# ly27253/LED-Net

Measured on AMD Instinct MI355X. Metric: images/sec at 1024x1024, LED-Net fwd+bwd, higher is better.
Workload: dtype bf16; 1 GPU; LED-Net 1024x1024 train_step (fwd+OHEM-CE+bwd+SGD) batch 16/GPU; global_batch=16, parallelism=dp1, ranks=1, batchnorm=per-rank statistics, submission=hipGraph replay, deterministic=False

## Files before the change

include/ledn.h:

```cpp
#ifndef LEDN_H
#define LEDN_H

#ifdef __cplusplus
extern "C" {
#endif

#define LEDN_ABI_VERSION 5

enum { LEDN_OK = 0, LEDN_EINVAL = 1, LEDN_ELAUNCH = 2, LEDN_ESKIP = 3  };
enum { LEDN_F32 = 0, LEDN_BF16 = 1, LEDN_U8 = 2 };
enum { LEDN_ACT_NONE = 0, LEDN_ACT_RELU = 1, LEDN_ACT_RELU6 = 2, LEDN_ACT_PRELU = 3, LEDN_ACT_SIGMOID = 4 };
enum { LEDN_RES_NONE = 0, LEDN_RES_ADD = 1, LEDN_RES_GATE = 2 };

int ledn_abi_version(void);

int ledn_set_workspace(void* ptr, long long nfloats);
int ledn_bind_workspace(void* stream, void* ptr, long long nfloats);

enum {
    LEDN_OPT_CONV_WORKGROUPS = 0,
    LEDN_OPT_WGRAD_WORKGROUPS = 1,
    LEDN_OPT_STREAM_FAST = 2,
    LEDN_OPT_BN_FUSED = 4,
    LEDN_OPT_DETERMINISTIC = 3
};
int ledn_set_option(int option, long long value);

typedef struct {
    const void* x;
    const void* xadd;
    const float* w;
    const void* w_bf16;
    void* y;
    const void* res;
    const float* in_scale;
    const float* in_shift;
    const float* out_scale;
    const float* out_shift;
    const float* slope;
    float* stat_sum;
    float* stat_sqsum;
    long long ws_co, ws_ci, ws_tap;
    int N, H, W, Cin, Ho, Wo, Cout;
    int KH, KW, stride, pad, dil, groups;
    int in_act, act_out, res_mode;
    int dtype_x, dtype_y;
    int transposed;
    const float* in_slope;
} ledn_conv_desc;
int ledn_conv2d(const ledn_conv_desc* d, void* stream);
int ledn_conv2d_deferred_stats(const ledn_conv_desc* d, float** part, int* rows, void* stream);
int ledn_stats_defer_begin(void);
int ledn_stats_defer_end(float** part, int* rows);
int ledn_conv2d_uses_mfma(const ledn_conv_desc* d);

int ledn_pack_conv_weights(const float* w, void* out_bf16, int Cout, int Cin, int KH, int KW, int mode,
// ... 242 lines not shown
int ledn_bn_act_bwd_reduce(const ledn_bnbwd_desc* d, void* stream);
int ledn_bn_act_bwd_apply(const ledn_bnbwd_desc* d, void* stream);
int ledn_bn_act_bwd_fused(const ledn_bnbwd_desc* d, void* stream);
int ledn_bn_act_bwd_fused_check(int C, void* stream);

typedef struct {
    ledn_bnbwd_desc bn;
    const void* head_dz;
    const float* w;
    float* dw;
    float* db;
    int N, H, W, Co;
    int dtype_dz;
} ledn_headbwd_desc;
int ledn_head_bwd_supported(const ledn_headbwd_desc* d);
int ledn_head_bwd_reduce(const ledn_headbwd_desc* d, void* stream);
int ledn_head_bwd_apply(const ledn_headbwd_desc* d, void* stream);

typedef struct {
    const void* x;
    const void* dz;
    const float* w;
    const void* add;
    void* dx;
    float* dw;
    int N, H, W, C, Ho, Wo;
    int KH, KW, stride, pad;
    int dil[4], group_size;
    int ext1;
    int dtype;
} ledn_dwbwd_desc;
int ledn_dwconv2d_bwd_data(const ledn_dwbwd_desc* d, void* stream);
int ledn_dwconv2d_bwd_weight(const ledn_dwbwd_desc* d, void* stream);

typedef struct {
    const void* x;
    const void* dy;
    const float* w;
    void* gsum;
    void* dx;
    float* dw;
    int N, H, W, n, Ho, Wo, stride;
    int dil[4];
    int dtype;
} ledn_pyrbwd_desc;
int ledn_sesp_pyramid_bwd_data(const ledn_pyrbwd_desc* d, void* stream);
int ledn_sesp_pyramid_bwd_weight(const ledn_pyrbwd_desc* d, void* stream);
int ledn_sesp_pyramid_bwd_kernel_id(const ledn_pyrbwd_desc* d);

int ledn_bilinear_bwd(const void* dy, void* dx, int N, int H, int W, int C, int Ho, int Wo,
                      int dtype_dy, int dtype_dx, void* stream);
int ledn_avgpool3x3s2_bwd(const void* dy, const void* add, void* dx, int N, int H, int W, int C,
                          int Ho, int Wo, int dtype, void* stream);

int ledn_window_attn_bwd(const void* qkv, const float* biasT, const void* dout, float* dqkv,
                         float* dbiasT, int N, int H, int W, int C, int heads, int ws, int dtype,
                         void* stream);
int ledn_getb_pool_bwd(const void* dout, void* da, int N, int H, int W, int C, int ws, int dtype,
                       void* stream);

typedef struct {
    const void* x;
    const void* r;
    const void* xl;
    const float* ctx[4];
    int ctx_size[4];
// ... 244 lines not shown
```

led-net_amd/_lib.py:

```python
import contextlib
import ctypes as C
import os

_HERE = os.path.dirname(os.path.abspath(__file__))
from ._env import knob as _knob
HIP_LIB_PATH = _knob('LEDN_HIP_LIB', None) or os.path.join(_HERE, 'csrc', 'libledn_hip.so')

OK, EINVAL, ELAUNCH = 0, 1, 2
F32, BF16, U8 = 0, 1, 2
ACT_NONE, ACT_RELU, ACT_RELU6, ACT_PRELU, ACT_SIGMOID = 0, 1, 2, 3, 4
RES_NONE, RES_ADD, RES_GATE = 0, 1, 2
OPT_CONV_WORKGROUPS, OPT_WGRAD_WORKGROUPS, OPT_STREAM_FAST, OPT_DETERMINISTIC, OPT_BN_FUSED = 0, 1, 2, 3, 4
ESKIP = 3

vp, fp, i32, i64 = C.c_void_p, C.c_void_p, C.c_int, C.c_longlong


class ConvDesc(C.Structure):
    _fields_ = [('x', vp), ('xadd', vp), ('w', fp), ('w_bf16', vp), ('y', vp), ('res', vp),
                ('in_scale', fp), ('in_shift', fp), ('out_scale', fp), ('out_shift', fp),
                ('slope', fp), ('stat_sum', fp), ('stat_sqsum', fp),
                ('ws_co', i64), ('ws_ci', i64), ('ws_tap', i64),
                ('N', i32), ('H', i32), ('W', i32), ('Cin', i32), ('Ho', i32), ('Wo', i32), ('Cout', i32),
                ('KH', i32), ('KW', i32), ('stride', i32), ('pad', i32), ('dil', i32), ('groups', i32),
                ('in_act', i32), ('act_out', i32), ('res_mode', i32),
                ('dtype_x', i32), ('dtype_y', i32), ('transposed', i32), ('in_slope', fp)]


class WgradDesc(C.Structure):
    _fields_ = [('x', vp), ('xadd', vp), ('dz', vp), ('dw', fp), ('db', fp),
                ('in_scale', fp), ('in_shift', fp),
                ('ws_co', i64), ('ws_ci', i64), ('ws_tap', i64),
                ('N', i32), ('H', i32), ('W', i32), ('Cin', i32), ('Ho', i32), ('Wo', i32), ('Cout', i32),
                ('KH', i32), ('KW', i32), ('stride', i32), ('pad', i32), ('dil', i32), ('groups', i32),
                ('in_act', i32), ('dtype_x', i32), ('dtype_dz', i32), ('in_slope', fp)]


class WgradFinishEntry(C.Structure):
    _fields_ = [('part', fp), ('dw', fp), ('ws_co', i64), ('ws_ci', i64), ('ws_tap', i64),
                ('nbx', i32), ('pairs', i32), ('KK', i32), ('ci_tiles', i32), ('Cin', i32), ('Cout', i32),
                ('groups', i32), ('chunk0', i32)]


class DwDesc(C.Structure):
    _fields_ = [('x', vp), ('w', fp), ('y', vp), ('out_scale', fp), ('out_shift', fp), ('slope', fp),
# ... 113 lines not shown
    _fields_ = [('w', fp), ('out', vp), ('Cout', i32), ('Cin', i32), ('KK', i32), ('mode', i32), ('groups', i32)]


class SgdEntry(C.Structure):
    _fields_ = [('p', fp), ('g', fp), ('m', fp), ('n', i64)]


class OptimEntry(C.Structure):
    _fields_ = [('p', fp), ('g', fp), ('m', fp), ('v', fp), ('n', i64), ('lr_mult', C.c_float), ('wd_mult', C.c_float)]


class EmaEntry(C.Structure):
    _fields_ = [('avg', fp), ('src', fp), ('n', i64)]


class OptimDesc(C.Structure):
    _fields_ = [('kind', i32), ('has_v', i32), ('lr_a', C.c_float), ('lr_b', C.c_float), ('sched_dev', fp),
                ('momentum', C.c_float), ('eps', C.c_float), ('beta1', C.c_double), ('beta2', C.c_double),
                ('bc1', C.c_float), ('sqrt_bc2', C.c_float), ('weight_decay', C.c_float), ('grad_scale', C.c_float),
                ('clip', i32), ('norm_type', i32), ('partials', fp), ('n_partials', i32), ('max_norm', C.c_float),
                ('clip_value', C.c_float), ('norm_out', fp)]


_PROTOS = {
    'ledn_bn_act_bwd_reduce': ([C.POINTER(BnBwdDesc), vp], i32),
    'ledn_bn_act_bwd_apply': ([C.POINTER(BnBwdDesc), vp], i32),
    'ledn_head_bwd_supported': ([C.POINTER(HeadBwdDesc)], i32),
    'ledn_head_bwd_reduce': ([C.POINTER(HeadBwdDesc), vp], i32),
    'ledn_head_bwd_apply': ([C.POINTER(HeadBwdDesc), vp], i32),
    'ledn_bn_act_bwd_fused': ([C.POINTER(BnBwdDesc), vp], i32),
    'ledn_bn_act_bwd_fused_check': ([i32, vp], i32),
    'ledn_dwconv2d_bwd_data': ([C.POINTER(DwBwdDesc), vp], i32),
    'ledn_dwconv2d_bwd_weight': ([C.POINTER(DwBwdDesc), vp], i32),
    'ledn_sesp_pyramid_bwd_data': ([C.POINTER(PyrBwdDesc), vp], i32),
    'ledn_sesp_pyramid_bwd_weight': ([C.POINTER(PyrBwdDesc), vp], i32),
    'ledn_sesp_pyramid_bwd_kernel_id': ([C.POINTER(PyrBwdDesc)], i32),
    'ledn_bilinear_bwd': ([vp, vp, i32, i32, i32, i32, i32, i32, i32, i32, vp], i32),
    'ledn_avgpool3x3s2_bwd': ([vp, vp, vp, i32, i32, i32, i32, i32, i32, i32, vp], i32),
    'ledn_window_attn_bwd': ([vp, fp, vp, fp, fp, i32, i32, i32, i32, i32, i32, i32, vp], i32),
    'ledn_getb_pool_bwd': ([vp, vp, i32, i32, i32, i32, i32, i32, vp], i32),
    'ledn_mfaf_gate_bwd': ([C.POINTER(MfafBwdDesc), vp], i32),
    'ledn_mfaf_bwd_combine': ([vp, vp, vp, C.POINTER(fp), C.POINTER(i32), i32, i32, i32, i32, i32, i32, vp], i32),
    'ledn_ohem_work_floats': ([i64], i64),
    'ledn_ohem_ce_fwd': ([fp, vp, i64, i32, C.c_float, i64, C.c_float, i32, fp, fp, vp], i32),
    'ledn_ohem_ce_bwd': ([fp, vp, i64, i32, i32, fp, fp, fp, C.c_float, fp, vp], i32),
    'ledn_ohem_ce_up_fwd': ([fp, i32, i32, i32, i32, i32, vp, C.c_float, i64, C.c_float, i32, fp, fp, vp], i32),
    'ledn_ohem_ce_up_bwd': ([fp, i32, i32, i32, i32, i32, vp, i32, fp, fp, fp, C.c_float, fp, vp], i32),
    'ledn_ohem2_up_fwd': ([fp, fp, i32, i32, i32, i32, i32, vp, C.c_float, i64, C.c_float, C.c_float, i64, C.c_float, i32,
                           fp, fp, vp], i32),
    'ledn_ohem2_up_bwd': ([fp, fp, i32, i32, i32, i32, i32, i32, fp, fp, fp, fp, C.c_float, C.c_float, fp, fp, vp], i32),
    'ledn_ohem2_work_floats': ([i64], i64),
    'ledn_ohem_ce_w_fwd': ([fp, vp, i64, i32, C.c_float, i64, C.c_float, i32, fp, fp, fp, vp], i32),
    'ledn_ohem_ce_w_bwd': ([fp, vp, i64, i32, i32, fp, fp, fp, C.c_float, fp, fp, vp], i32),
    'ledn_ohem_ce_up_w_fwd': ([fp, i32, i32, i32, i32, i32, vp, C.c_float, i64, C.c_float, i32, fp, fp, fp, vp], i32),
    'ledn_ohem_ce_up_w_bwd': ([fp, i32, i32, i32, i32, i32, vp, i32, fp, fp, fp, C.c_float, fp, fp, vp], i32),
    'ledn_ohem2_up_w_fwd': ([fp, fp, i32, i32, i32, i32, i32, vp, C.c_float, i64, C.c_float, C.c_float, i64, C.c_float, i32,
                             fp, fp, fp, fp, vp], i32),
    'ledn_ohem2_up_w_bwd': ([fp, fp, i32, i32, i32, i32, i32, i32, fp, fp, fp, fp, C.c_float, C.c_float, fp, fp, fp, fp,
                             vp], i32),
    'ledn_seg_loss_work_floats': ([i64], i64),
    'ledn_ce_loss_fwd': ([fp, vp, i32, i64, i32, fp, i32, i32, i32, C.c_float, fp, fp, vp], i32),
    'ledn_ce_loss_bwd': ([fp, vp, i32, i64, i32, fp, i32, C.c_float, fp, fp, fp, fp, vp], i32),
    'ledn_ce_loss_up_fwd': ([fp, i32, i32, i32, i32, i32, vp, fp, i32, i32, i32, C.c_float, fp, fp, vp], i32),
    'ledn_ce_loss_up_bwd': ([fp, i32, i32, i32, i32, i32, vp, fp, i32, C.c_float, fp, fp, fp, fp, vp], i32),
    'ledn_dice_loss_fwd': ([fp, vp, i32, i64, i32, i32, i32, i32, i32, i32, C.c_float, C.c_float, fp, fp, vp], i32),
    'ledn_dice_loss_bwd': ([fp, vp, i32, i64, i32, i32, i32, i32, i32, C.c_float, C.c_float, fp, fp, fp, fp, vp], i32),
# ... 167 lines not shown
```

led-net_amd/csrc/backward.hip:

```cpp
#include "ledn_rt.h"
#include "stencil.h"

namespace ledn {

template <int V>
struct BnParams {
    float sc[V], sh[V], sl[V], mean[V], invstd[V];
};

template <int V>
__device__ __forceinline__ BnParams<V> bn_params(const ledn_bnbwd_desc& d, int c) {
    BnParams<V> p;
#pragma unroll
    for (int i = 0; i < V; ++i) {
        p.sc[i] = d.scale ? d.scale[c + i] : 1.f;
        p.sh[i] = d.shift ? d.shift[c + i] : 0.f;
        p.sl[i] = d.slope ? d.slope[c + i] : 0.f;
        p.mean[i] = d.bn_mode ? d.mean[c + i] : 0.f;
        p.invstd[i] = d.bn_mode ? d.invstd[c + i] : 0.f;
    }
    return p;
}

template <int V>
// ... 563 lines not shown
        if (!part && nbx > 64) {
            ppb = cdiv(cdiv(npix, 64), rows) * rows;
            nbx = cdiv(npix, ppb);
        }
        const dim3 g8((unsigned)nbx, (unsigned)d.KH);
        if (d.dtype == LEDN_F32) LEDN_LAUNCH((dw_bwd_weight_row_kernel<float, 4, 8>), g8, dim3(256), 0, s, d, (int)ppb, part);
        else if (d.dtype == LEDN_BF16) LEDN_LAUNCH((dw_bwd_weight_row_kernel<bf16_t, 4, 8>), g8, dim3(256), 0, s, d, (int)ppb, part);
        else return LEDN_EINVAL;
        if (part) return finish_partials(part, (int)nbx, d.KH * 8 * d.C, 1, d.dw, nullptr, nullptr, s);
        return check_launch();
    }
    const int taps = d.KH * d.KW;
    long ppb = cdiv(npix * taps, 8192);
    if (ppb < 128) ppb = 128;
    long nbx = cdiv(npix, ppb);
    float* part = (nbx > 8 || det()) ? ws_take(nbx * taps * d.C) : nullptr;
    if (!part) {
        ppb = cdiv(npix * taps, 2048);
        if (ppb < 128) ppb = 128;
        nbx = cdiv(npix, ppb);
    }
    const dim3 grid((unsigned)nbx, (unsigned)taps);
#define LEDN_K(T)                                                                                       \
    do {                                                                                                \
        if (v4) LEDN_LAUNCH((dw_bwd_weight_kernel<T, 4>), grid, dim3(256), 0, s, d, (int)ppb, part);    \
        else LEDN_LAUNCH((dw_bwd_weight_kernel<T, 1>), grid, dim3(256), 0, s, d, (int)ppb, part);       \
    } while (0)
    if (d.dtype == LEDN_F32) LEDN_K(float);
    else if (d.dtype == LEDN_BF16) LEDN_K(bf16_t);
    else return LEDN_EINVAL;
#undef LEDN_K
    if (part) return finish_partials(part, (int)nbx, taps * d.C, 1, d.dw, nullptr, nullptr, s);
    return check_launch();
}

template <typename T, int V>
__global__ void __launch_bounds__(256) pyr_suffix_kernel(const T* dy, T* g, long npix, int n) {
    const int cv = n / V;
    const long idx = (long)blockIdx.x * blockDim.x + threadIdx.x;
    if (idx >= npix * cv) return;
    const int c = (int)(idx % cv) * V;
    const long pix = idx / cv;
    float run[V];
#pragma unroll
    for (int v = 0; v < V; ++v) run[v] = 0.f;
    for (int b = 3; b >= 0; --b) {
        float t[V];
        ldv<V>(dy + pix * 4L * n + (long)b * n + c, t);
#pragma unroll
        for (int v = 0; v < V; ++v) run[v] += t[v];
        stv<V>(g + pix * 4L * n + (long)b * n + c, run);
    }
}

template <typename T, int V>
__global__ void __launch_bounds__(256) pyr_bwd_data_kernel(ledn_pyrbwd_desc d) {
    const int cv = d.n / V;
    const long total = (long)d.N * d.H * d.W * cv;
    const long idx = (long)xcd_block(blockIdx.x, gridDim.x) * blockDim.x + threadIdx.x;
    if (idx >= total) return;
    const NhwcIdx ix_ = nhwc_split(idx, cv, d.W, d.H);
    const int c = ix_.cv * V;
    const long pix = ix_.pix;
    const int x = ix_.x, y = ix_.y, n = ix_.n;
    const T* g = reinterpret_cast<const T*>(d.gsum);
    float acc[V];
// ... 800 lines not shown
```

led-net_amd/csrc/capi.hip:

```cpp
#include "ledn_rt.h"

namespace ledn {
int conv_validate(const ledn_conv_desc& d);
int conv_direct(const ledn_conv_desc& d, hipStream_t s);
bool conv_mfma_supported(const ledn_conv_desc& d);
bool conv_f32_mfma_supported(const ledn_conv_desc& d);
int conv_f32_mfma(const ledn_conv_desc& d, hipStream_t s);
bool conv_wgrad_f32_mfma_supported(const ledn_wgrad_desc& d);
int conv_wgrad_f32_mfma(const ledn_wgrad_desc& d, hipStream_t s);
int conv_mfma(const ledn_conv_desc& d, hipStream_t s);
int conv_wgrad_mfma_partial(const ledn_wgrad_desc& d, float* part, long long part_floats, ledn_wgrad_finish_entry* entry,
                            bool query, hipStream_t s);
int conv_wgrad_finish_multi_impl(const ledn_wgrad_finish_entry* table_dev, int n, int total_chunks, hipStream_t s);
bool conv1x1_reg_supported(const ledn_conv_desc& d);
int conv1x1_reg(const ledn_conv_desc& d, hipStream_t s);
bool conv3x3_reg_supported(const ledn_conv_desc& d);
int conv3x3_reg(const ledn_conv_desc& d, hipStream_t s);
bool conv3x3_narrowin_mfma_supported(const ledn_conv_desc& d);
int conv3x3_narrowin_mfma(const ledn_conv_desc& d, hipStream_t s);
bool wgrad_mfma_supported(const ledn_wgrad_desc& d);
bool conv_wgrad_cout2_supported(const ledn_wgrad_desc& d);
bool conv_wgrad_narrow_reg_supported(const ledn_wgrad_desc& d);
bool conv1x1_wgrad_reg_applies(const ledn_wgrad_desc& d);
int conv_wgrad_narrow_reg(const ledn_wgrad_desc& d, hipStream_t s);
// ... 34 lines not shown
int channel_stats_impl(const void* x, const void* xadd, long long P, int C, int dtype, float* sum,
                       float* sqsum, hipStream_t s);
int bn_finalize_impl(const float* sum, const float* sqsum, double count, const float* gamma,
                     const float* beta, float* running_mean, float* running_var, float momentum,
                     float eps, float* scale, float* shift, float* mean, float* invstd, int C,
                     hipStream_t s);
int affine_act_impl(const ledn_affine_desc& d, hipStream_t s);
int bilinear_impl(const ledn_resize_desc& d, hipStream_t s);
int nchw_to_nhwc_impl(const void* x, int dtype_x, void* y, int dtype_y, int N, int C, int H, int W,
                      const float* scale, const float* shift, const int* map, const int* valid_hw, float pad_val,
                      hipStream_t s);
int avgpool2d_impl(const void* x, void* y, int N, int H, int W, int C, int Ho, int Wo, int k, int st, int pad,
                   int dtype, hipStream_t s);
int avgpool2d_bwd_impl(const void* dy, void* dx, int N, int H, int W, int C, int Ho, int Wo, int k, int st, int pad,
                       int dtype, hipStream_t s);
int relpos_bias_impl(const float* table, const long long* index, float* out, int R, int heads, int T, hipStream_t s);
int relpos_bias_bwd_impl(const float* dbias, const long long* index, float* dtable, int R, int heads, int T,
                         hipStream_t s);
int adaptive_avgpool_impl(const void* x, const void* xadd, float* y, int N, int H, int W, int C, int S,
                          int dtype, hipStream_t s);
int avgpool3x3s2_impl(const void* x, void* y, int N, int H, int W, int C, int Ho, int Wo, int dtype,
                      hipStream_t s);
int window_attn_impl(const void* qkv, const float* biasT, void* out, int N, int H, int W, int C,
                     int heads, int ws, int dtype, hipStream_t s);
int getb_pool_impl(const void* a, const void* local, void* out, int N, int H, int W, int C, int ws,
                   int dtype, hipStream_t s);
int mfaf_gate_impl(const ledn_mfaf_desc& d, hipStream_t s);
int seam_edge_impl(const float* seg, float* edge, float* scratch, int N, int h, int w, int kth, float thr,
                   float final_thr, hipStream_t s);
int bn_act_bwd_reduce_impl(const ledn_bnbwd_desc& d, hipStream_t s);
int bn_act_bwd_apply_impl(const ledn_bnbwd_desc& d, hipStream_t s);
int dw_bwd_data_impl(const ledn_dwbwd_desc& d, hipStream_t s);
int dw_bwd_weight_impl(const ledn_dwbwd_desc& d, hipStream_t s);
int pyr_bwd_data_impl(const ledn_pyrbwd_desc& d, hipStream_t s);
int pyr_bwd_weight_impl(const ledn_pyrbwd_desc& d, hipStream_t s);
int pyr_bwd_data_kernel_id(const ledn_pyrbwd_desc& d);
int bilinear_bwd_impl(const void* dy, void* dx, int N, int H, int W, int C, int Ho, int Wo, int dtype_dy,
                      int dtype_dx, hipStream_t s);
int avgpool3x3s2_bwd_impl(const void* dy, const void* add, void* dx, int N, int H, int W, int C, int Ho,
                          int Wo, int dtype, hipStream_t s);
int window_attn_bwd_impl(const void* qkv, const float* biasT, const void* dout, float* dqkv, float* dbiasT,
                         int N, int H, int W, int C, int heads, int ws, int dtype, hipStream_t s);
int getb_pool_bwd_impl(const void* dout, void* da, int N, int H, int W, int C, int ws, int dtype,
                       hipStream_t s);
int mfaf_gate_bwd_impl(const ledn_mfafbwd_desc& d, hipStream_t s);
int mfaf_bwd_combine_impl(void* dx, void* dr, const void* dxl, const float* const* dpool, const int* sizes,
                          int npool, int N, int H, int W, int C, int dtype, hipStream_t s);
long long ohem_work_floats(long long P);
int ohem_ce_fwd_impl(const float* logits, const long long* target, long long P, int C, float thres,
                     long long min_kept, float loss_weight, int ignore_label, const float* cw, float* work,
                     float* out, hipStream_t s);
int ohem_ce_up_fwd_impl(const float* src, int N, int Hs, int Ws, int H, int W, const long long* target, float thres,
                        long long min_kept, float loss_weight, int ignore_label, const float* cw, float* work,
                        float* out, hipStream_t s);
int ohem2_up_fwd_impl(const float* src0, const float* src1, int N, int Hs, int Ws, int H, int W,
                      const long long* target, float thres0, long long min_kept0, float lw0, float thres1,
                      long long min_kept1, float lw1, int ignore_label, const float* cw0, const float* cw1,
                      float* work, float* out, hipStream_t s);
int ohem2_up_bwd_impl(const float* src0, const float* src1, int N, int Hs, int Ws, int H, int W, int ignore_label,
                      const float* work, const float* out, const float* dloss0, const float* dloss1, float lw0,
                      float lw1, const float* cw0, const float* cw1, float* dsrc0, float* dsrc1, hipStream_t s);
long long ohem2_work_floats(long long P);
int ohem_ce_up_bwd_impl(const float* src, int N, int Hs, int Ws, int H, int W, const long long* target,
                        int ignore_label, const float* work, const float* out, const float* dloss, float loss_weight,
                        const float* cw, float* dsrc, hipStream_t s);
int ohem_ce_bwd_impl(const float* logits, const long long* target, long long P, int C, int ignore_label,
// ... 20 lines not shown
int slide_accumulate_impl(float* canvas, const float* crop, int N, int C, int H, int W, int y1, int x1, int hc, int wc,
                          int crop_planar, hipStream_t s);
int slide_finish_impl(float* canvas, const int* rowcnt, const int* colcnt, unsigned char* mask, int N, int C, int H,
                      int W, hipStream_t s);
int sgd_step_impl(const ledn_sgd_entry* table_dev, int n_tensors, long long max_n, float lr,
                  const float* lr_dev, float momentum, float weight_decay, float grad_scale, hipStream_t s);
int grad_norm_partials_impl(const float* g, long long n, int norm_type, float* partials, int n_partials, hipStream_t s);
int sgd_step_clip_impl(const ledn_sgd_entry* table_dev, int n_tensors, long long max_n, float lr, const float* lr_dev,
                       float momentum, float weight_decay, float grad_scale, const float* partials, int n_partials,
                       int norm_type, float max_norm, float clip_value, float* norm_out, hipStream_t s);
int optim_step_impl(const ledn_optim_entry* table_dev, int n_tensors, long long max_n, const ledn_optim_desc* d, hipStream_t s);
int optim_step_ema_impl(const ledn_optim_entry* table_dev, float* const* avg_table_dev, int n_tensors, long long max_n,
                        const ledn_optim_desc* d, float w, const float* w_dev, hipStream_t s);
int ema_update_impl(const ledn_ema_entry* table_dev, int n_tensors, long long max_n, float w, const float* w_dev, hipStream_t s);
}

#include <mutex>
#include <unordered_map>

namespace ledn {
static Workspace g_ws = {nullptr, 0};
static std::mutex g_ws_mutex;
static std::unordered_map<void*, Workspace> g_ws_by_stream;
static thread_local void* tls_stream = nullptr;
static thread_local Workspace tls_ws = {nullptr, 0};
static hipStream_t enter_stream(void* stream) {
    tls_stream = stream;
    std::lock_guard<std::mutex> lock(g_ws_mutex);
    auto it = g_ws_by_stream.find(stream);
    tls_ws = it != g_ws_by_stream.end() ? it->second : g_ws;
    return (hipStream_t)stream;
}
Workspace& workspace() { return tls_ws; }
static Options g_opt = {512, 512, 91, 0, 0};
Options& options() { return g_opt; }
static thread_local DeferredStats g_defer = {false, nullptr, 0};
DeferredStats& deferred_stats() { return g_defer; }
}

using namespace ledn;
#define S(stream) (ledn::enter_stream(stream))

extern "C" {

int ledn_abi_version(void) { return LEDN_ABI_VERSION; }

int ledn_set_workspace(void* ptr, long long nfloats) {
    if (nfloats < 0 || (ptr == nullptr) != (nfloats == 0)) return LEDN_EINVAL;
    std::lock_guard<std::mutex> lock(g_ws_mutex);
    g_ws = Workspace{(float*)ptr, (long)nfloats};
    if (g_ws_by_stream.find(tls_stream) == g_ws_by_stream.end()) tls_ws = g_ws;
    return LEDN_OK;
}

int ledn_bind_workspace(void* stream, void* ptr, long long nfloats) {
    if (nfloats < 0 || (ptr == nullptr) != (nfloats == 0)) return LEDN_EINVAL;
    std::lock_guard<std::mutex> lock(g_ws_mutex);
    if (ptr) g_ws_by_stream[stream] = Workspace{(float*)ptr, (long)nfloats};
    else g_ws_by_stream.erase(stream);
    return LEDN_OK;
}

int ledn_set_option(int option, long long value) {
    if (value > (1 << 20)) return LEDN_EINVAL;
    switch (option) {
        case LEDN_OPT_CONV_WORKGROUPS: options().conv_workgroups = value > 0 ? (int)value : 512; return LEDN_OK;
        case LEDN_OPT_WGRAD_WORKGROUPS: options().wgrad_workgroups = value > 0 ? (int)value : 512; return LEDN_OK;
        case LEDN_OPT_STREAM_FAST: options().stream_fast = value < 0 ? 91 : (int)value; return LEDN_OK;
        case LEDN_OPT_DETERMINISTIC: options().deterministic = value > 0 ? 1 : 0; return LEDN_OK;
        case LEDN_OPT_BN_FUSED: options().bn_fused = value > 0 ? 1 : 0; return LEDN_OK;
        default: return LEDN_EINVAL;
    }
}

int ledn_conv2d(const ledn_conv_desc* d, void* stream) {
    if (!d) return LEDN_EINVAL;
    const int rc = conv_validate(*d);
    if (rc != LEDN_OK) return rc;
    if (head_fwd_supported(*d)) return head_fwd(*d, S(stream));
    if (head_mc_conv_kind(*d)) return head_mc_conv(*d, S(stream));
    if (conv_mfma_supported(*d)) {
        if (conv1x1_reg_supported(*d)) return conv1x1_reg(*d, S(stream));
        if (conv3x3_reg_supported(*d)) return conv3x3_reg(*d, S(stream));
        return conv_mfma(*d, S(stream));
    }
    if (conv3x3_narrowin_mfma_supported(*d)) return conv3x3_narrowin_mfma(*d, S(stream));
    if (conv_f32_mfma_supported(*d)) return conv_f32_mfma(*d, S(stream));
    return conv_direct(*d, S(stream));
}

int ledn_stats_defer_begin(void) {
    DeferredStats& ds = deferred_stats();
    ds.want = true;
    ds.part = nullptr;
    ds.rows = 0;
    return LEDN_OK;
}
int ledn_stats_defer_end(float** part, int* rows) {
    if (!part || !rows) return LEDN_EINVAL;
    DeferredStats& ds = deferred_stats();
    *part = ds.part;
    *rows = ds.part ? ds.rows : 0;
    ds.want = false;
// ... 226 lines not shown
int ledn_mfaf_gate(const ledn_mfaf_desc* d, void* stream) { return d ? mfaf_gate_impl(*d, S(stream)) : LEDN_EINVAL; }
int ledn_seam_edge(const float* seg, float* edge, float* scratch, int N, int h, int w, int kth, float thr,
                   float final_thr, void* stream) {
    return seam_edge_impl(seg, edge, scratch, N, h, w, kth, thr, final_thr, S(stream));
}

int ledn_bn_act_bwd_reduce(const ledn_bnbwd_desc* d, void* stream) {
    return d ? bn_act_bwd_reduce_impl(*d, S(stream)) : LEDN_EINVAL;
}
int ledn_bn_act_bwd_apply(const ledn_bnbwd_desc* d, void* stream) {
    return d ? bn_act_bwd_apply_impl(*d, S(stream)) : LEDN_EINVAL;
}
int ledn_bn_act_bwd_fused(const ledn_bnbwd_desc* d, void* stream) {
    if (!d) return LEDN_EINVAL;
    if (!options().bn_fused) return LEDN_ESKIP;
    return bn_act_bwd_fused(*d, S(stream));
}
int ledn_bn_act_bwd_fused_check(int C, void* stream) { return bn_act_bwd_fused_check(C, S(stream)); }
int ledn_head_bwd_supported(const ledn_headbwd_desc* d) { return d ? head_bwd_supported(*d) : 0; }
int ledn_head_bwd_reduce(const ledn_headbwd_desc* d, void* stream) {
    LEDN_REQUIRE(d);
    return head_bwd_reduce(*d, S(stream));
}
int ledn_head_bwd_apply(const ledn_headbwd_desc* d, void* stream) {
    LEDN_REQUIRE(d);
    return head_bwd_apply(*d, S(stream));
}
int ledn_dwconv2d_bwd_data(const ledn_dwbwd_desc* d, void* stream) {
    return d ? dw_bwd_data_impl(*d, S(stream)) : LEDN_EINVAL;
}
int ledn_dwconv2d_bwd_weight(const ledn_dwbwd_desc* d, void* stream) {
    return d ? dw_bwd_weight_impl(*d, S(stream)) : LEDN_EINVAL;
}
int ledn_sesp_pyramid_bwd_data(const ledn_pyrbwd_desc* d, void* stream) {
    return d ? pyr_bwd_data_impl(*d, S(stream)) : LEDN_EINVAL;
}
int ledn_sesp_pyramid_bwd_weight(const ledn_pyrbwd_desc* d, void* stream) {
    return d ? pyr_bwd_weight_impl(*d, S(stream)) : LEDN_EINVAL;
}
int ledn_sesp_pyramid_bwd_kernel_id(const ledn_pyrbwd_desc* d) { return d ? pyr_bwd_data_kernel_id(*d) : -1; }
int ledn_bilinear_bwd(const void* dy, void* dx, int N, int H, int W, int C, int Ho, int Wo, int dtype_dy,
                      int dtype_dx, void* stream) {
    return bilinear_bwd_impl(dy, dx, N, H, W, C, Ho, Wo, dtype_dy, dtype_dx, S(stream));
}
int ledn_avgpool3x3s2_bwd(const void* dy, const void* add, void* dx, int N, int H, int W, int C, int Ho,
                          int Wo, int dtype, void* stream) {
    return avgpool3x3s2_bwd_impl(dy, add, dx, N, H, W, C, Ho, Wo, dtype, S(stream));
}
int ledn_window_attn_bwd(const void* qkv, const float* biasT, const void* dout, float* dqkv, float* dbiasT,
                         int N, int H, int W, int C, int heads, int ws, int dtype, void* stream) {
    return window_attn_bwd_impl(qkv, biasT, dout, dqkv, dbiasT, N, H, W, C, heads, ws, dtype, S(stream));
}
int ledn_getb_pool_bwd(const void* dout, void* da, int N, int H, int W, int C, int ws, int dtype,
                       void* stream) {
    return getb_pool_bwd_impl(dout, da, N, H, W, C, ws, dtype, S(stream));
}
int ledn_mfaf_gate_bwd(const ledn_mfafbwd_desc* d, void* stream) {
    return d ? mfaf_gate_bwd_impl(*d, S(stream)) : LEDN_EINVAL;
}
int ledn_mfaf_bwd_combine(void* dx, void* dr, const void* dxl, const float* const* dpool, const int* sizes,
                          int npool, int N, int H, int W, int C, int dtype, void* stream) {
    return mfaf_bwd_combine_impl(dx, dr, dxl, dpool, sizes, npool, N, H, W, C, dtype, S(stream));
}
long long ledn_ohem_work_floats(long long P) { return ohem_work_floats(P); }
int ledn_ohem_ce_fwd(const float* logits, const long long* target, long long P, int C, float thres,
                     long long min_kept, float loss_weight, int ignore_label, float* work, float* out,
// ... 243 lines not shown
```

led-net_amd/csrc/dwconv.hip:

```cpp
#include "ledn_rt.h"
#include "stencil.h"

namespace ledn {

template <typename TX, typename TY, int V, int KK>
__global__ void __launch_bounds__(256) dwconv_kernel(ledn_dw_desc d, float* part) {
    __shared__ float s_part[2][256 * 4];
    const int cvn = d.C / V;
    const int rows = 256 / cvn;
    const int r = threadIdx.x / cvn, cv = threadIdx.x % cvn;
    const int c = cv * V;
    float st1[V], st2[V];
#pragma unroll
    for (int v = 0; v < V; ++v) st1[v] = st2[v] = 0.f;
    if (r < rows) {
        const int dl = d.dil[c / d.group_size];
        const int padh = d.pad >= 0 ? d.pad : dl * (d.KH - 1) / 2;
        const int padw = d.pad >= 0 ? d.pad : dl * (d.KW - 1) / 2;
        const int Hx = d.H + (d.ext1 ? 1 : 0), Wx = d.W + (d.ext1 ? 1 : 0);
        const TX* x = reinterpret_cast<const TX*>(d.x);
        float wreg[KK > 0 ? KK : 1][V];
        if (KK > 0) {
#pragma unroll
            for (int t = 0; t < KK; ++t) ldv<V>(d.w + (long)t * d.C + c, wreg[t]);
// ... 646 lines not shown
static bool dw3x3_bf16_ok(int C, int group_size, int KH, int KW, int stride, int pad, int ext1, const int* dil,
                          long numel) {
    if (KH != 3 || KW != 3 || stride != 1 || ext1 || C % 8 || group_size % 8 || 256 % (C / 8) || C / 8 > 256) return false;
    if (numel >= (1L << 31)) return false;
    for (int g = 0; g * group_size < C; ++g)
        if (pad >= 0 && pad != dil[g]) return false;
    return true;
}

int dw3x3_bwd_data_bf16(const ledn_dwbwd_desc& b, hipStream_t s) {
    if (b.dtype != LEDN_BF16 || !dw3x3_bf16_ok(b.C, b.group_size, b.KH, b.KW, b.stride, b.pad, b.ext1, b.dil,
                                               (long)b.N * b.H * b.W * b.C))
        return -1;
    ledn_dw_desc d = {};
    d.x = b.dz; d.w = b.w; d.y = b.dx;
    d.N = b.N; d.H = b.H; d.W = b.W; d.C = b.C; d.Ho = b.H; d.Wo = b.W;
    d.KH = d.KW = 3; d.stride = 1; d.pad = b.pad; d.group_size = b.group_size;
    for (int i = 0; i < 4; ++i) d.dil[i] = b.dil[i];
    if (options().stream_fast & 2) {
        float* part = nullptr;
        long rows = 0;
        if (dw3x3_tile_launch(d, true, (const bf16_t*)b.add, false, &part, &rows, s) == 0) return check_launch();
    }
    const int rows = 256 / (d.C / 8);
    long nb = cdiv((long)d.N * d.H * d.W, rows * 4);
    if (nb > 2048) nb = 2048;
    LEDN_LAUNCH((dw3x3_bf16_kernel<1>), dim3((unsigned)nb), dim3(256), 0, s, d, (const bf16_t*)b.add, (float*)nullptr);
    return check_launch();
}

int finish_partials(const float* part, int nblk, int C, int nout, float* o0, float* o1, float* o2,
                    hipStream_t s);

int dwconv_impl(const ledn_dw_desc& d, hipStream_t s) {
    LEDN_REQUIRE(d.x && d.w && d.y);
    LEDN_REQUIRE(d.N > 0 && d.H > 0 && d.W > 0 && d.C > 0 && d.Ho > 0 && d.Wo > 0);
    LEDN_REQUIRE(d.KH > 0 && d.KW > 0 && d.stride > 0 && d.group_size > 0);
    LEDN_REQUIRE(d.C <= 512 && d.C <= 4 * d.group_size);
    LEDN_REQUIRE((d.stat_sum == nullptr) == (d.stat_sqsum == nullptr));
    LEDN_REQUIRE(d.act_out != LEDN_ACT_PRELU || d.slope != nullptr);
    LEDN_REQUIRE(!d.ext1 || (d.H >= 2 && d.W >= 2));
    for (int g = 0; g * d.group_size < d.C; ++g) {
        LEDN_REQUIRE(d.dil[g] > 0);
        const int Hx = d.H + (d.ext1 ? 1 : 0), Wx = d.W + (d.ext1 ? 1 : 0);
        const int ph = d.pad >= 0 ? d.pad : d.dil[g] * (d.KH - 1) / 2;
        const int pw = d.pad >= 0 ? d.pad : d.dil[g] * (d.KW - 1) / 2;
        LEDN_REQUIRE(d.Ho == (Hx + 2 * ph - ((d.KH - 1) * d.dil[g] + 1)) / d.stride + 1);
        LEDN_REQUIRE(d.Wo == (Wx + 2 * pw - ((d.KW - 1) * d.dil[g] + 1)) / d.stride + 1);
    }
    if (dw8x8_tile_ok(d)) {
        const long tiles = (long)d.N * cdiv(d.Ho, 8) * cdiv(d.Wo, 32);
        float* part = nullptr;
        if (d.stat_sum) part = ws_take(tiles * 2 * d.C);
        if (!d.stat_sum || part) {
            LEDN_LAUNCH((dw8x8_tile_kernel<0>), dim3((unsigned)(tiles * (d.C / 32))), dim3(256), 0, s, d, part, 3);
            if (part) return finish_partials(part, (int)tiles, d.C, 2, d.stat_sum, d.stat_sqsum, nullptr, s);
            return check_launch();
        }
    }
    if (d.dtype_x == LEDN_BF16 && d.dtype_y == LEDN_BF16 && d.act_out != LEDN_ACT_SIGMOID && d.Ho == d.H &&
        d.Wo == d.W &&
        dw3x3_bf16_ok(d.C, d.group_size, d.KH, d.KW, d.stride, d.pad, d.ext1, d.dil, (long)d.N * d.H * d.W * d.C)) {
        if (options().stream_fast & 2) {
            float* partt = nullptr;
            long rowst = 0;
            if (dw3x3_tile_launch(d, false, nullptr, d.stat_sum != nullptr, &partt, &rowst, s) == 0) {
// ... 184 lines not shown
```

led-net_amd/csrc/ledn_rt.h:

```cpp
#pragma once
#include <stdint.h>

#ifdef LEDN_CPU_EMU
#include "emu.h"
#else
#include <hip/hip_runtime.h>
#define LEDN_LAUNCH(kernel, grid, block, smem, stream, ...) \
    hipLaunchKernelGGL(kernel, grid, block, smem, stream, __VA_ARGS__)
#endif

#include "../../include/ledn.h"

namespace ledn {

struct bf16_t {
    unsigned short v;
};

__device__ __forceinline__ float bf16_to_f32(unsigned short b) { return __uint_as_float(((unsigned)b) << 16); }
#ifdef LEDN_CPU_EMU
__device__ __forceinline__ unsigned short f32_to_bf16(float f) {
    unsigned u = __float_as_uint(f);
    if ((u & 0x7fffffffu) > 0x7f800000u) return (unsigned short)((u >> 16) | 0x0040u);
    u += 0x7fffu + ((u >> 16) & 1u);
// ... 301 lines not shown
__device__ __forceinline__ void sched_fence() { __builtin_amdgcn_sched_barrier(0); }
typedef __bf16 hw_bf16x8_t __attribute__((ext_vector_type(8)));
__device__ __forceinline__ f32x16_t mfma_32x32x16_bf16(bf16x8_t a, bf16x8_t b, f32x16_t c) {
    return __builtin_amdgcn_mfma_f32_32x32x16_bf16(__builtin_bit_cast(hw_bf16x8_t, a),
                                                   __builtin_bit_cast(hw_bf16x8_t, b), c, 0, 0, 0);
}
__device__ __forceinline__ bf16x4_t lds_read_tr16(const void* p) {
    return __builtin_amdgcn_ds_read_tr16_b64_v4i16(
        (__attribute__((address_space(3))) bf16x4_t*)(const_cast<void*>(p)));
}
#endif

inline int check_launch() {
    hipError_t e = hipGetLastError();
    return e == hipSuccess ? LEDN_OK : LEDN_ELAUNCH;
}
__host__ __device__ inline long cdiv(long a, long b) { return (a + b - 1) / b; }

struct Workspace {
    float* ptr;
    long nfloats;
};
Workspace& workspace();
inline float* ws_take(long nfloats) {
    Workspace& w = workspace();
    return (w.ptr && nfloats <= w.nfloats) ? w.ptr : nullptr;
}
struct Options {
    int conv_workgroups;
    int wgrad_workgroups;
    int stream_fast;
    int deterministic;
    int bn_fused;
};
Options& options();
inline long exp_knob(const char* name, long def) {
    const char* e = getenv("LEDN_EXPERIMENTAL");
    const char* v = (e && atoi(e)) ? getenv(name) : nullptr;
    return v ? atol(v) : def;
}
inline bool det() { return options().deterministic != 0; }
struct DeferredStats {
    bool want;
    float* part;
    int rows;
};
DeferredStats& deferred_stats();
int finish_partials(const float* part, int nblk, int C, int nout, float* o0, float* o1, float* o2,
                    hipStream_t s);
int affine_act_fast(const ledn_affine_desc& d, hipStream_t s);
int bn_act_bwd_reduce_fast(const ledn_bnbwd_desc& d, hipStream_t s);
int bn_act_bwd_apply_fast(const ledn_bnbwd_desc& d, hipStream_t s);
int bn_act_bwd_fused(const ledn_bnbwd_desc& d, hipStream_t s);
int bn_act_bwd_fused_check(int C, hipStream_t s);
int head_bwd_supported(const ledn_headbwd_desc& d);
int head_bwd_reduce(const ledn_headbwd_desc& d, hipStream_t s);
int head_bwd_apply(const ledn_headbwd_desc& d, hipStream_t s);
bool head_fwd_supported(const ledn_conv_desc& d);
int head_fwd(const ledn_conv_desc& d, hipStream_t s);
int head_mc_conv_kind(const ledn_conv_desc& d);
int head_mc_conv(const ledn_conv_desc& d, hipStream_t s);
bool head_mc_wgrad_supported(const ledn_wgrad_desc& d);
int head_mc_wgrad(const ledn_wgrad_desc& d, hipStream_t s);
int channel_stats_fast(const void* x, const void* xadd, long long P, int C, int dtype, float* sum, float* sqsum,
                       hipStream_t s);
enum { SL_CE = 0, SL_DICE_SIGMOID = 1, SL_DICE_SOFTMAX = 2, SL_FOCAL = 3, SL_TVERSKY = 4 };
// ... 22 lines not shown
```

led-net_amd/ops_train.py:

```python
import ctypes as C
import math

import torch

from . import _lib
from . import ops as _ops
from .ops import (ACT_NONE, RES_NONE, _DT, LednError, _check, _dt, _f32, _nb, _p, _run,
                  conv_out_size)


class _BnBwd:
    __slots__ = ('lib', 'd', 'z', 'bn', 'Cc', 'P', 'local', 'sunk', 'dz', 'dres', 'dslope', 'slope_sunk', 'keep', 'reduce_pending', 'hd')


from ._env import knob_int as _knob_int
BN_ROWS = _knob_int('LEDN_BN_ROWS', 0)


def bn_act_bwd_reduce(z, dy, *, scale=None, shift=None, mean=None, invstd=None, act=ACT_NONE, slope=None,
                      res=None, res_mode=RES_NONE, count=None, want_dres=False, sinks=None, sync=False,
                      dz_add=None, dres_add=None, launch=True, head=None, no_dz=False):
    lib = _lib.get_lib()
    st = _BnBwd()
    Cc = z.shape[-1]
# ... 166 lines not shown
                and w.shape[0] == 2 and w.shape[1] == 32 and x.shape[-1] == 32 and stride == 1 and pad == 1
                and groups == 1 and act in (ACT_NONE, _ops.ACT_RELU, _ops.ACT_PRELU) and x.numel() // x.shape[-1] >= 16384
                and x.numel() < (1 << 31) and dz.shape[1:3] == x.shape[1:3])


DW_WGRAD_SLOT = _knob_int('LEDN_DW_WGRAD_SLOT', 0)


def _on_side_stream(ref, sink, *keep):
    import contextlib
    if not (DW_WGRAD_SLOT and _ops.MULTI_STREAM and ref.is_cuda and sink is not None and _ops._slot(ref) == 0):
        return contextlib.nullcontext()
    cur = torch.cuda.current_stream(ref.device)
    side = _ops._aux_stream(ref.device, DW_WGRAD_SLOT)
    side.wait_stream(cur)
    for t in keep:
        if isinstance(t, torch.Tensor):
            t.record_stream(side)
    return torch.cuda.stream(side)


def _dw_desc(x_shape, dz, w_khwc, stride, pad, dil, group_size, ext1, dtype):
    N, H, W, Cc = x_shape
    KH, KW, _ = w_khwc.shape
    d = _lib.DwBwdDesc()
    d.N, d.H, d.W, d.C, d.Ho, d.Wo = N, H, W, Cc, dz.shape[1], dz.shape[2]
    d.KH, d.KW, d.stride, d.pad = KH, KW, stride, pad
    for i in range(4):
        d.dil[i] = dil[i] if i < len(dil) else dil[-1]
    d.group_size, d.ext1, d.dtype = group_size or Cc, int(ext1), dtype
    return d


def dwconv2d_bwd(x, dz, w_khwc, *, stride=1, pad=-1, dil=(1, 1, 1, 1), group_size=None, ext1=False,
                 add=None, need_dx=True, need_dw=True, dw_out=None):
    lib = _lib.get_lib()
    if dz.dtype != x.dtype:
        raise LednError('dwconv2d_bwd: dz dtype must match x')
    dx = dw = None
    d = _dw_desc(x.shape, dz, w_khwc, stride, pad, dil, group_size, ext1, _dt(x))
    _check(lib, x, dz, w_khwc, add)
    d.x, d.dz, d.w, d.add = _p(x), _p(dz), _p(_f32(w_khwc)), _p(add)
    KH, KW, Cc = w_khwc.shape
    if need_dx:
        dx = torch.empty_like(x)
        d.dx = _p(dx)
        _run(lib, 'ledn_dwconv2d_bwd_data', x, d, work=_ops._TIMING is not None and (f'dwbwd_data{KH}x{KW} C{Cc} {tuple(x.shape)}', _nb(dz, dx, add), 2 * dz.numel() * KH * KW))
    if need_dw:
        dw = dw_out if dw_out is not None else _ops.zeros_f32(tuple(w_khwc.shape), x.device)
        if tuple(dw.shape) != tuple(w_khwc.shape) or dw.dtype != torch.float32:
            raise LednError('dwconv2d_bwd: dw_out shape/dtype mismatch')
        _check(lib, dw)
        d.dw = _p(dw)
        with _on_side_stream(x, dw_out, x, dz, dw):
            _run(lib, 'ledn_dwconv2d_bwd_weight', x, d, work=_ops._TIMING is not None and (f'dwbwd_w{KH}x{KW} C{Cc} {tuple(x.shape)}', _nb(x, dz) , 2 * dz.numel() * KH * KW))
    return dx, dw


def _dwpack_desc(lib, weights, stacked, sinks=None):
    d = _lib.DwPackDesc()
    if not 0 < len(weights) <= 8:
        raise LednError('dw pack: 1..8 filters')
    KH, KW = weights[0].shape[2:]
    for k, w in enumerate(weights):
        if w.dim() != 4 or w.shape[1] != 1 or tuple(w.shape[2:]) != (KH, KW) or w.dtype != torch.float32:
            raise LednError('dw pack: depthwise filters [n,1,KH,KW] f32 of one kernel size expected')
        if stacked and w.shape[0] != weights[0].shape[0]:
            raise LednError('dw pack: stacked banks need equal channel counts')
        _check(lib, w)
        d.w[k], d.n[k] = w.data_ptr(), w.shape[0]
        if sinks is not None:
            g = sinks[k]
            if g.shape != w.shape or g.dtype != torch.float32:
                raise LednError('dw pack: gradient sink shape/dtype mismatch')
            _check(lib, g)
            d.dw[k] = g.data_ptr()
# ... 994 lines not shown
```

Measured before the change: 1346 images/s.

## Fuse depthwise 3x3 backward data and weight gradients into one tiled kernel

Adds a bf16 depthwise 3x3 backward kernel that stages a dz tile with halo in shared memory once. From that tile it computes both dx (including the optional residual add) and per-workgroup weight-gradient partials, which are then reduced by finish_partials. The goal is to avoid reading dz twice and launching separate data and weight kernels for the 3x3 dilated depthwise convolutions. It adds a new workgroup-count option and a Python fast path, which is used only when the dw-grad is not sent to a side stream. In exchange it loses the overlap the side-stream wgrad provided and needs a partials workspace.

```diff
diff --git a/include/ledn.h b/include/ledn.h
--- a/include/ledn.h
+++ b/include/ledn.h
@@ -22,6 +22,7 @@
     LEDN_OPT_WGRAD_WORKGROUPS = 1,
     LEDN_OPT_STREAM_FAST = 2,
     LEDN_OPT_BN_FUSED = 4,
+    LEDN_OPT_DW_BWD_WORKGROUPS = 5,
     LEDN_OPT_DETERMINISTIC = 3
 };
 int ledn_set_option(int option, long long value);
@@ -330,6 +331,8 @@
 } ledn_dwbwd_desc;
 int ledn_dwconv2d_bwd_data(const ledn_dwbwd_desc* d, void* stream);
 int ledn_dwconv2d_bwd_weight(const ledn_dwbwd_desc* d, void* stream);
+int ledn_dwconv2d_bwd(const ledn_dwbwd_desc* d, void* stream);
+int ledn_dwconv2d_bwd_fused_applies(const ledn_dwbwd_desc* d);
 
 typedef struct {
     const void* x;
diff --git a/led-net_amd/_lib.py b/led-net_amd/_lib.py
--- a/led-net_amd/_lib.py
+++ b/led-net_amd/_lib.py
@@ -11,6 +11,7 @@
 ACT_NONE, ACT_RELU, ACT_RELU6, ACT_PRELU, ACT_SIGMOID = 0, 1, 2, 3, 4
 RES_NONE, RES_ADD, RES_GATE = 0, 1, 2
 OPT_CONV_WORKGROUPS, OPT_WGRAD_WORKGROUPS, OPT_STREAM_FAST, OPT_DETERMINISTIC, OPT_BN_FUSED = 0, 1, 2, 3, 4
+OPT_DW_BWD_WORKGROUPS = 5
 ESKIP = 3
 
 vp, fp, i32, i64 = C.c_void_p, C.c_void_p, C.c_int, C.c_longlong
@@ -190,6 +191,8 @@
     'ledn_bn_act_bwd_fused_check': ([i32, vp], i32),
     'ledn_dwconv2d_bwd_data': ([C.POINTER(DwBwdDesc), vp], i32),
     'ledn_dwconv2d_bwd_weight': ([C.POINTER(DwBwdDesc), vp], i32),
+    'ledn_dwconv2d_bwd': ([C.POINTER(DwBwdDesc), vp], i32),
+    'ledn_dwconv2d_bwd_fused_applies': ([C.POINTER(DwBwdDesc)], i32),
     'ledn_sesp_pyramid_bwd_data': ([C.POINTER(PyrBwdDesc), vp], i32),
     'ledn_sesp_pyramid_bwd_weight': ([C.POINTER(PyrBwdDesc), vp], i32),
     'ledn_sesp_pyramid_bwd_kernel_id': ([C.POINTER(PyrBwdDesc)], i32),
diff --git a/led-net_amd/csrc/backward.hip b/led-net_amd/csrc/backward.hip
--- a/led-net_amd/csrc/backward.hip
+++ b/led-net_amd/csrc/backward.hip
@@ -619,6 +619,18 @@
 #undef LEDN_K
     if (part) return finish_partials(part, (int)nbx, taps * d.C, 1, d.dw, nullptr, nullptr, s);
     return check_launch();
+}
+
+int dw3x3_bwd_fused(const ledn_dwbwd_desc& b, hipStream_t s);
+
+int dw_bwd_impl(const ledn_dwbwd_desc& d, hipStream_t s) {
+    int rc = dwbwd_validate(d);
+    if (rc != LEDN_OK) return rc;
+    LEDN_REQUIRE(d.x && d.w && d.dx && d.dw);
+    rc = dw3x3_bwd_fused(d, s);
+    if (rc >= 0) return rc;
+    rc = dw_bwd_data_impl(d, s);
+    return rc != LEDN_OK ? rc : dw_bwd_weight_impl(d, s);
 }
 
 template <typename T, int V>
diff --git a/led-net_amd/csrc/capi.hip b/led-net_amd/csrc/capi.hip
--- a/led-net_amd/csrc/capi.hip
+++ b/led-net_amd/csrc/capi.hip
@@ -90,6 +90,8 @@
 int bn_act_bwd_apply_impl(const ledn_bnbwd_desc& d, hipStream_t s);
 int dw_bwd_data_impl(const ledn_dwbwd_desc& d, hipStream_t s);
 int dw_bwd_weight_impl(const ledn_dwbwd_desc& d, hipStream_t s);
+int dw_bwd_impl(const ledn_dwbwd_desc& d, hipStream_t s);
+bool dw3x3_bwd_fused_applies(const ledn_dwbwd_desc& b);
 int pyr_bwd_data_impl(const ledn_pyrbwd_desc& d, hipStream_t s);
 int pyr_bwd_weight_impl(const ledn_pyrbwd_desc& d, hipStream_t s);
 int pyr_bwd_data_kernel_id(const ledn_pyrbwd_desc& d);
@@ -176,7 +178,7 @@
     return (hipStream_t)stream;
 }
 Workspace& workspace() { return tls_ws; }
-static Options g_opt = {512, 512, 91, 0, 0};
+static Options g_opt = {512, 512, 91, 0, 0, 512};
 Options& options() { return g_opt; }
 static thread_local DeferredStats g_defer = {false, nullptr, 0};
 DeferredStats& deferred_stats() { return g_defer; }
@@ -213,6 +215,7 @@
         case LEDN_OPT_STREAM_FAST: options().stream_fast = value < 0 ? 91 : (int)value; return LEDN_OK;
         case LEDN_OPT_DETERMINISTIC: options().deterministic = value > 0 ? 1 : 0; return LEDN_OK;
         case LEDN_OPT_BN_FUSED: options().bn_fused = value > 0 ? 1 : 0; return LEDN_OK;
+        case LEDN_OPT_DW_BWD_WORKGROUPS: options().dw_bwd_workgroups = value > 0 ? (int)value : 512; return LEDN_OK;
         default: return LEDN_EINVAL;
     }
 }
@@ -505,6 +508,8 @@
 int ledn_dwconv2d_bwd_weight(const ledn_dwbwd_desc* d, void* stream) {
     return d ? dw_bwd_weight_impl(*d, S(stream)) : LEDN_EINVAL;
 }
+int ledn_dwconv2d_bwd(const ledn_dwbwd_desc* d, void* stream) { return d ? dw_bwd_impl(*d, S(stream)) : LEDN_EINVAL; }
+int ledn_dwconv2d_bwd_fused_applies(const ledn_dwbwd_desc* d) { return d && dw3x3_bwd_fused_applies(*d) ? 1 : 0; }
 int ledn_sesp_pyramid_bwd_data(const ledn_pyrbwd_desc* d, void* stream) {
     return d ? pyr_bwd_data_impl(*d, S(stream)) : LEDN_EINVAL;
 }
diff --git a/led-net_amd/csrc/dwconv.hip b/led-net_amd/csrc/dwconv.hip
--- a/led-net_amd/csrc/dwconv.hip
+++ b/led-net_amd/csrc/dwconv.hip
@@ -702,6 +702,153 @@
 int finish_partials(const float* part, int nblk, int C, int nout, float* o0, float* o1, float* o2,
                     hipStream_t s);
 
+template <int HL, int TH>
+__global__ void __launch_bounds__(256, 2) dw3x3_bwd_tile_kernel(ledn_dwbwd_desc d, float* part, int R) {
+    constexpr int TW = 32, PW = TW + 2 * HL, PH = TH + 2 * HL, CW = 32, PXB = CW * 2;
+    constexpr int NL = (PH * PW * 4 + 255) / 256;
+    __shared__ __attribute__((aligned(16))) unsigned char s_patch[PH * PW * PXB];
+    static_assert(PH * PW * PXB >= 4 * 9 * CW * 4, "the weight-gradient exchange reuses the patch");
+    float* s_red = reinterpret_cast<float*>(s_patch);
+    const int tid = threadIdx.x;
+    const int tx = (d.W + TW - 1) / TW, ty = (d.H + TH - 1) / TH, nch = d.C / CW;
+    const int tiles = d.N * tx * ty;
+    const unsigned bid = xcd_block(blockIdx.x, gridDim.x);
+    const int ch = (int)(bid % (unsigned)nch), row = (int)(bid / (unsigned)nch);
+    const int cg = tid & 3, pl = tid >> 2;
+    const int c = ch * CW + cg * 8;
+    const int dl = d.dil[c / d.group_size];
+    f32x2_t w[9][4], acc[9][4];
+    int toff[9];
+#pragma unroll
+    for (int t = 0; t < 9; ++t) {
+        f32x8_load(d.w + (long)(8 - t) * d.C + c, w[t]);
+        toff[t] = (((t / 3 - 1) * dl) * PW + (t % 3 - 1) * dl) * PXB;
+#pragma unroll
+        for (int i = 0; i < 4; ++i) acc[t][i] = f32x2_t{0.f, 0.f};
+    }
+    const int lx = pl & 31;
+    for (int tile = row; tile < tiles; tile += R) {
+        const int txi = tile % tx, tyi = (tile / tx) % ty, n = tile / (tx * ty);
+        const int y0 = tyi * TH - HL, x0 = txi * TW - HL;
+        const long img = (long)n * d.H * d.W * d.C;
+        const bf16_t* zin = reinterpret_cast<const bf16_t*>(d.dz) + img + ch * CW;
+        const bf16_t* xin = reinterpret_cast<const bf16_t*>(d.x) + img + c;
+        bf16_t* y = reinterpret_cast<bf16_t*>(d.dx) + img + c;
+        const bf16_t* addp = d.add ? reinterpret_cast<const bf16_t*>(d.add) + img + c : nullptr;
+        const int gx = txi * TW + lx;
+        const int gy0 = tyi * TH + (pl >> 5);
+        auto request = [&](int pass, uint4& xr, uint4& ar) {
+            const int gy = gy0 + pass * 2;
+            if (pass < TH / 2 && gy < d.H && gx < d.W) {
+                const unsigned o = (unsigned)((gy * d.W + gx) * d.C);
+                xr = *reinterpret_cast<const uint4*>(xin + o);
+                if (addp) ar = *reinterpret_cast<const uint4*>(addp + o);
+            }
+        };
+        uint4 xa = {0u, 0u, 0u, 0u}, xb = xa, aa = xa, ab = xa;
+        request(0, xa, aa);
+        request(1, xb, ab);
+        {
+            const int tid_o = opaque(tid);
+            uint4 stage[NL];
+#pragma unroll
+            for (int i = 0; i < NL; ++i) {
+                const int e = tid_o + i * 256, px = e >> 2, q = e & 3;
+                const int gy = y0 + px / PW, gx = x0 + px % PW;
+                const bool ok = e < PH * PW * 4 && gy >= 0 && gy < d.H && gx >= 0 && gx < d.W;
+                const unsigned off = ok ? (unsigned)((gy * d.W + gx) * d.C + q * 8) : 0u;
+                const uint4 v = *reinterpret_cast<const uint4*>(zin + off);
+                stage[i] = ok ? v : uint4{0u, 0u, 0u, 0u};
+            }
+#pragma unroll
+            for (int i = 0; i < NL; ++i) {
+                const int e = tid_o + i * 256;
+                if (e < PH * PW * 4) *reinterpret_cast<uint4*>(s_patch + (long)e * 16) = stage[i];
+            }
+        }
+        __syncthreads();
+        auto do_pass = [&](int pass, uint4& xr, uint4& ar) {
+            const int ly = pass * 2 + (pl >> 5), gy = gy0 + pass * 2;
+            f32x2_t dxv[4], xc[4];
+            bf16x8_unpack(ar, dxv);
+            bf16x8_unpack(xr, xc);
+            request(pass + 2, xr, ar);
+            if (gy >= d.H || gx >= d.W) return;
+            const unsigned o = (unsigned)((gy * d.W + gx) * d.C);
+            const unsigned char* ctr = s_patch + ((ly + HL) * PW + lx + HL) * PXB + cg * 16;
+            uint4 raw[9];
+#pragma unroll
+            for (int t = 0; t < 9; ++t) raw[t] = *reinterpret_cast<const uint4*>(ctr + toff[t]);
+#pragma unroll
+            for (int t = 0; t < 9; ++t) {
+                f32x2_t zv[4];
+                bf16x8_unpack(raw[t], zv);
+#pragma unroll
+                for (int i = 0; i < 4; ++i) {
+                    dxv[i] = pk_fma(zv[i], w[t][i], dxv[i]);
+                    acc[t][i] = pk_fma(zv[i], xc[i], acc[t][i]);
+                }
+            }
+            *reinterpret_cast<uint4*>(y + o) = bf16x8_pack(dxv);
+        };
+#pragma unroll 1
+        for (int pass = 0; pass < TH / 2; pass += 2) {
+            do_pass(pass, xa, aa);
+            do_pass(pass + 1, xb, ab);
+        }
+        __syncthreads();
+    }
+    f32x2_t s[9];
+#pragma unroll
+    for (int t = 0; t < 9; ++t) {
+        swap_add32(acc[t][0], acc[t][1]);
+        swap_add32(acc[t][2], acc[t][3]);
+        swap_add16(acc[t][0], acc[t][2]);
+        s[t].x = lane_step_sum(lane_step_sum(acc[t][0].x, 4), 8);
+        s[t].y = lane_step_sum(lane_step_sum(acc[t][0].y, 4), 8);
+    }
+    const int lane = tid & 63, wid = tid >> 6, rr = lane >> 4;
+    if ((lane & 15) < 4) {
+        const int cc = cg * 8 + 2 * (2 * (rr & 1) + (rr >> 1));
+#pragma unroll
+        for (int t = 0; t < 9; ++t)
+            *reinterpret_cast<float2*>(s_red + (wid * 9 + 8 - t) * CW + cc) = make_float2(s[t].x, s[t].y);
+    }
+    __syncthreads();
+    for (int e = tid; e < 9 * CW; e += 256) {
+        const float sum = (s_red[e] + s_red[9 * CW + e]) + (s_red[18 * CW + e] + s_red[27 * CW + e]);
+        part[(long)row * 9 * d.C + (long)(e / CW) * d.C + ch * CW + e % CW] = sum;
+    }
+}
+
+bool dw3x3_bwd_fused_applies(const ledn_dwbwd_desc& b) {
+    if (b.dtype != LEDN_BF16 || b.Ho != b.H || b.Wo != b.W || b.C <= 0 || b.group_size <= 0 || b.C > 4 * b.group_size ||
+        !dw3x3_bf16_ok(b.C, b.group_size, b.KH, b.KW, b.stride, b.pad, b.ext1, b.dil, (long)b.N * b.H * b.W * b.C))
+        return false;
+    if (b.C % 32 || b.W < 32 || (long)b.N * b.H * b.W < 16384) return false;
+    int hl = 0;
+    for (int g = 0; g * b.group_size < b.C; ++g) {
+        if (b.dil[g] < 1) return false;
+        hl = b.dil[g] > hl ? b.dil[g] : hl;
+    }
+    if (hl > 5) return false;
+    return (long)b.N * cdiv(b.H, hl <= 2 ? 16 : 8) * cdiv(b.W, 32) <= 16384;
+}
+
+int dw3x3_bwd_fused(const ledn_dwbwd_desc& b, hipStream_t s) {
+    if (!(options().stream_fast & 2) || !dw3x3_bwd_fused_applies(b)) return -1;
+    int hl = 0;
+    for (int g = 0; g * b.group_size < b.C; ++g) hl = b.dil[g] > hl ? b.dil[g] : hl;
+    const int nch = b.C / 32;
+    long R = options().dw_bwd_workgroups / nch;
+    R = R < 1 ? 1 : R > 256 ? 256 : R;
+    float* part = ws_take(R * 9 * b.C);
+    if (!part) return -1;
+    if (hl <= 2) LEDN_LAUNCH((dw3x3_bwd_tile_kernel<2, 16>), dim3((unsigned)(R * nch)), dim3(256), 0, s, b, part, (int)R);
+    else LEDN_LAUNCH((dw3x3_bwd_tile_kernel<5, 8>), dim3((unsigned)(R * nch)), dim3(256), 0, s, b, part, (int)R);
+    return finish_partials(part, (int)R, 9 * b.C, 1, b.dw, nullptr, nullptr, s);
+}
+
 int dwconv_impl(const ledn_dw_desc& d, hipStream_t s) {
     LEDN_REQUIRE(d.x && d.w && d.y);
     LEDN_REQUIRE(d.N > 0 && d.H > 0 && d.W > 0 && d.C > 0 && d.Ho > 0 && d.Wo > 0);
diff --git a/led-net_amd/csrc/ledn_rt.h b/led-net_amd/csrc/ledn_rt.h
--- a/led-net_amd/csrc/ledn_rt.h
+++ b/led-net_amd/csrc/ledn_rt.h
@@ -357,6 +357,7 @@
     int stream_fast;
     int deterministic;
     int bn_fused;
+    int dw_bwd_workgroups;
 };
 Options& options();
 inline long exp_knob(const char* name, long def) {
diff --git a/led-net_amd/ops_train.py b/led-net_amd/ops_train.py
--- a/led-net_amd/ops_train.py
+++ b/led-net_amd/ops_train.py
@@ -222,6 +222,11 @@
     return d
 
 
+def dwconv2d_bwd_fused_applies(x, dz, w_khwc, *, stride=1, pad=-1, dil=(1, 1, 1, 1), group_size=None, ext1=False):
+    d = _dw_desc(x.shape, dz, w_khwc, stride, pad, dil, group_size, ext1, _dt(x))
+    return bool(_lib.get_lib().cdll.ledn_dwconv2d_bwd_fused_applies(d))
+
+
 def dwconv2d_bwd(x, dz, w_khwc, *, stride=1, pad=-1, dil=(1, 1, 1, 1), group_size=None, ext1=False,
                  add=None, need_dx=True, need_dw=True, dw_out=None):
     lib = _lib.get_lib()
@@ -232,6 +237,21 @@
     _check(lib, x, dz, w_khwc, add)
     d.x, d.dz, d.w, d.add = _p(x), _p(dz), _p(_f32(w_khwc)), _p(add)
     KH, KW, Cc = w_khwc.shape
+    side = DW_WGRAD_SLOT and _ops.MULTI_STREAM and x.is_cuda and dw_out is not None and _ops._slot(x) == 0
+    if need_dx and need_dw and not side:
+        dx = torch.empty_like(x)
+        dw = dw_out if dw_out is not None else _ops.zeros_f32(tuple(w_khwc.shape), x.device)
+        if tuple(dw.shape) != tuple(w_khwc.shape) or dw.dtype != torch.float32:
+            raise LednError('dwconv2d_bwd: dw_out shape/dtype mismatch')
+        _check(lib, dw)
+        d.dx, d.dw = _p(dx), _p(dw)
+        work = None
+        if _ops._TIMING is not None:
+            work = (f'dwbwd{KH}x{KW} C{Cc} {tuple(x.shape)}', _nb(x, dz, dx, add), 4 * dz.numel() * KH * KW)
+            if lib.cdll.ledn_dwconv2d_bwd_fused_applies(d):
+                work += ('dw3x3_bwd_tile_kernel',)
+        _run(lib, 'ledn_dwconv2d_bwd', x, d, work=work)
+        return dx, dw
     if need_dx:
         dx = torch.empty_like(x)
         d.dx = _p(dx)
```

After: 1362 images/s (median of 6 runs). 1.2% higher.
